# maximyudayev/Realtime-ST-GCN

Measured on AMD Instinct MI355X. Metric: skeleton-frames/sec/GPU (fwd+bwd), 10-layer ST-GCN N=64 T=300 V=25, higher is better.
Workload: dtype bf16; 1 GPU; config 2: as_is st-gcn (fcn_in + 9 StgcnLayer, BatchNorm, Kt=9), fwd + loss + bwd + Adam; global_batch=64, seq_len=300, joints=25, parallelism=single, bn_stats=per-replica, launch=eager

## Files before the change

realtime-st-gcn_amd/csrc/gconv.hip:

```cpp
#include "common.h"
#include "lds_ops.h"
#include "pack.h"
#include <stdlib.h>
#include "../../include/stgcn_amd.h"

#ifndef GCONV_NSTG_N
#define GCONV_NSTG_N 2
#endif
#ifndef GCONV_NSTG_M
#define GCONV_NSTG_M 2
#endif
#ifndef GCONV_NSTG_W
#define GCONV_NSTG_W 2
#endif
#ifndef GCONV_TM_W
#define GCONV_TM_W 2
#endif
#ifndef GCONV_TM_M
#define GCONV_TM_M 1
#endif

namespace {

template <typename T, int KC>
// ... 96 lines not shown
    const long joff = (long)src * a.in_ld + c * KC;
    const int ci = c * KC + ucol * VEC;
#pragma unroll
    for (int u = 0; u < A_UNITS; ++u) {
      ra[u] = make_uint4(0, 0, 0, 0);
      if (a_row[u] >= 0) {
        const T* p = in + a_row[u] + joff;
        if (fast_ld) {
          ra[u] = *reinterpret_cast<const uint4*>(p);
        } else if (ci < a.Cin) {
          float f[VEC];
#pragma unroll
          for (int e = 0; e < VEC; ++e) f[e] = ci + e < a.Cin ? Tr<T>::to_f(p[e]) : 0.f;
          ra[u] = pack16(f, (T*)nullptr);
        }
      }
    }
    char* B_ = smem + buf * STAGE + A_BYTES;
    const T* wsrc = wp + ((long)(jt * a.J + j) * a.Cout_pad + n0) * a.Cin_pad + c * KC;
#pragma unroll
    for (int kk = 0; kk < (B_PIECES + NW - 1) / NW; ++kk) {
      const int piece = wave + kk * NW;
      if (piece < B_PIECES) {
        const int byte = piece * 1024 + lane * 16;
        const int br = byte / L::RB, pu = (byte % L::RB) >> 4;
        glds16(wsrc + (long)br * a.Cin_pad + (pu ^ L::swz(br)) * VEC, B_ + piece * 1024);
      }
    }
  };
  auto store = [&](int buf) {
    char* A_ = smem + buf * STAGE;
#pragma unroll
    for (int u = 0; u < A_UNITS; ++u) *reinterpret_cast<uint4*>(A_ + a_lds[u]) = ra[u];
  };

  f32x16 acc[TM][TN];
#pragma unroll
  for (int i = 0; i < TM; ++i)
#pragma unroll
    for (int j = 0; j < TN; ++j)
#pragma unroll
      for (int r = 0; r < 16; ++r) acc[i][j][r] = 0.f;

  typedef typename Tr<T>::frag Frag;
  if constexpr (NSTG > 0) {
    static_assert(sizeof(T) == 2 && KC == 64, "DMA K loop: bf16, 64-channel chunks");
    constexpr int RBD = 128, A_B = BM * RBD, STG = A_B + BN * RBD;
    constexpr int AI = BM / 8 / NW, BI = BN / 8 / NW, OPS = AI + BI;
    static_assert(BM % (8 * NW) == 0 && BN % (8 * NW) == 0, "DMA rows");
    int* const snbr = reinterpret_cast<int*>(smem + NSTG * STG);
    if (tid < a.J) snbr[tid] = a.nbr[jt * a.J + tid];
    __syncthreads();
    const int rr = lane >> 3, slot = lane & 7;
    long a_src[AI];
    int b_src[BI];
#pragma unroll
    for (int q = 0; q < AI; ++q) {
      const int r = (wave * AI + q) * 8 + rr;
      const int rc = min(r, max(rows_valid, 1) - 1);
      a_src[q] = (long)(i0 + rc) * V * a.in_ld + (slot ^ ((r >> 1) & 7)) * 8;
    }
#pragma unroll
    for (int q = 0; q < BI; ++q) {
      const int r = (wave * BI + q) * 8 + rr;
      b_src[q] = (n0 + r) * a.Cin_pad + (slot ^ ((r >> 1) & 7)) * 8;
    }
    auto issue = [&](int k, int stage) {
      const int j = k / nch, c = k - j * nch;
      const long joff = (long)snbr[j] * a.in_ld + c * KC;
      const T* wsrc = wp + (long)(jt * a.J + j) * a.Cout_pad * a.Cin_pad + c * KC;
      char* base = smem + stage * STG;
#pragma unroll
      for (int q = 0; q < AI; ++q) glds16(in + a_src[q] + joff, lds_u32(base + (wave * AI + q) * 1024));
#pragma unroll
      for (int q = 0; q < BI; ++q) glds16(wsrc + b_src[q], lds_u32(base + A_B + (wave * BI + q) * 1024));
    };
#pragma unroll
    for (int sidx = 0; sidx < NSTG - 1; ++sidx)
      if (sidx < nk) issue(sidx, sidx);
    for (int k = 0; k < nk; ++k) {
      const int younger = min(NSTG - 2, nk - 1 - k);
      gwait_vm(younger * OPS);
      asm volatile("s_waitcnt lgkmcnt(0)\n\ts_barrier" ::: "memory");
      if (k + NSTG - 1 < nk) issue(k + NSTG - 1, (k + NSTG - 1) % NSTG);
      const char* A_ = smem + (k % NSTG) * STG;
      const char* B_ = A_ + A_B;
#pragma unroll
      for (int ks = 0; ks < KS; ++ks) {
        Frag fa[TM], fb[TN];
#pragma unroll
        for (int i = 0; i < TM; ++i) {
          const int r = (wm * TM + i) * 32 + lr;
          fa[i] = __builtin_bit_cast(bf16x8, *reinterpret_cast<const uint4*>(A_ + r * RBD + (((2 * ks + lh) ^ ((r >> 1) & 7)) << 4)));
        }
#pragma unroll
        for (int j = 0; j < TN; ++j) {
          const int r = (wn * TN + j) * 32 + lr;
          fb[j] = __builtin_bit_cast(bf16x8, *reinterpret_cast<const uint4*>(B_ + r * RBD + (((2 * ks + lh) ^ ((r >> 1) & 7)) << 4)));
        }
#pragma unroll
        for (int i = 0; i < TM; ++i)
#pragma unroll
          for (int j = 0; j < TN; ++j) Tr<T>::mma(acc[i][j], fa[i], fb[j]);
      }
    }
    __syncthreads();
  } else {
  int cur = 0;
  if (nk > 0) {
    load(0, 0);
    store(0);
  }
  __syncthreads();
  for (int k = 0; k < nk; ++k) {
    const bool more = k + 1 < nk;
    if (more) load(k + 1, cur ^ 1);
    const char* A_ = smem + cur * STAGE;
    const char* B_ = A_ + A_BYTES;
    Frag fa[2][TM], fb[2][TN];
    auto rd = [&](int ks, int b) {
#pragma unroll
      for (int i = 0; i < TM; ++i) {
        const char* p = A_ + a_off[i] + ks * 16 * (int)sizeof(T);
        fa[b][i] = frag2<T>(p, p + 16);
      }
#pragma unroll
      for (int j = 0; j < TN; ++j) {
        const char* p = B_ + ((wn * TN + j) * 32) * L::RB;
        fb[b][j] = frag2<T>(p + b_off[ks][0], p + b_off[ks][1]);
      }
    };
    rd(0, 0);
#pragma unroll
    for (int ks = 0; ks < KS; ++ks) {
      if (ks + 1 < KS) rd(ks + 1, (ks + 1) & 1);
#pragma unroll
      for (int i = 0; i < TM; ++i)
#pragma unroll
        for (int j = 0; j < TN; ++j) Tr<T>::mma(acc[i][j], fa[ks & 1][i], fb[ks & 1][j]);
      __builtin_amdgcn_sched_barrier(0);
    }
    if (more) store(cur ^ 1);
    __syncthreads();
    cur ^= 1;
  }
  }

  T* __restrict__ out = reinterpret_cast<T*>(a.out);
  const long ldv = (long)a.out_ld * V;
  constexpr int SROW = 32 * (int)sizeof(T) + 16;
  constexpr int UR = 32 * (int)sizeof(T) / 16;
  char* scratch = smem + wave * 32 * SROW;
  constexpr bool vec_out = ACCV;
  Welford ws[TN];
#pragma unroll
  for (int j = 0; j < TN; ++j) {
    const int c0 = n0 + (wn * TN + j) * 32;
    const int col = c0 + lr;
    const bool cok = col < a.Cout;
    const float b1 = (a.bias && cok) ? a.bias[jt * a.Cout + col] : 0.f;
    float s = 0.f, cnt = 0.f;
    if constexpr (!vec_out) {
#pragma unroll
      for (int i = 0; i < TM; ++i) {
        const int lb = (wm * TM + i) * 32 + 4 * lh;
        T* pb = out + ((long)(i0 + lb) * V + jt) * a.out_ld + col;
#pragma unroll
        for (int r = 0; r < 16; ++r) {
          const int ro = (r & 3) + 8 * (r >> 2);
          const bool ok = cok && lb + ro < rows_valid;
          float v = acc[i][j][r] + b1;
          if (ok) {
            T* p = pb + ro * ldv;
            if (a.accumulate) v += Tr<T>::to_f(*p);
            *p = Tr<T>::from_f(v);
            s += v;
            cnt += 1.f;
          }
          acc[i][j][r] = v;
        }
      }
    } else {
#pragma unroll
      for (int i = 0; i < TM; ++i) {
        const int rb = (wm * TM + i) * 32;
        const int lb = rb + 4 * lh;
#pragma unroll
        for (int r = 0; r < 16; ++r) {
          const int ro = (r & 3) + 8 * (r >> 2);
          const float v = acc[i][j][r] + b1;
          acc[i][j][r] = v;
          if (cok && lb + ro < rows_valid) {
            s += v;
            cnt += 1.f;
          }
          *reinterpret_cast<T*>(scratch + (4 * lh + ro) * SROW + lr * (int)sizeof(T)) = Tr<T>::from_f(v);
        }
#pragma unroll
        for (int q = 0; q < 32 * UR / 64; ++q) {
          const int idx = q * 64 + lane, row = idx / UR, u = idx % UR;
          if (rb + row < rows_valid && c0 + u * VEC < a.Cout) {
            T* p = out + ((long)(i0 + rb + row) * V + jt) * a.out_ld + c0 + u * VEC;
            float f[VEC], o[VEC];
            if (a.accumulate) {
              unpack16(*reinterpret_cast<const uint4*>(scratch + row * SROW + u * 16), f, (T*)nullptr);
              unpack16(*reinterpret_cast<const uint4*>(p), o, (T*)nullptr);
#pragma unroll
              for (int e = 0; e < VEC; ++e) f[e] += o[e];
              *reinterpret_cast<uint4*>(p) = pack16(f, (T*)nullptr);
            } else if (sizeof(T) == 2 && a.res) {
              const long grow = (long)(i0 + rb + row) * V + jt;
              const int cc = c0 + u * VEC;
              unpack16(*reinterpret_cast<const uint4*>(scratch + row * SROW + u * 16), f, (T*)nullptr);
              unpack16(*reinterpret_cast<const uint4*>(reinterpret_cast<const T*>(a.res) + grow * a.res_ld + cc), o,
                       (T*)nullptr);
              const unsigned mb = reinterpret_cast<const unsigned char*>(a.res_bits)[grow * (a.Cout / 8) + cc / 8];
#pragma unroll
              for (int e = 0; e < VEC; ++e) f[e] += ((mb >> e) & 1u) ? o[e] : 0.f;
              *reinterpret_cast<uint4*>(p) = pack16(f, (T*)nullptr);
            } else {
              *reinterpret_cast<uint4*>(p) = *reinterpret_cast<const uint4*>(scratch + row * SROW + u * 16);
            }
          }
        }
      }
    }
    Welford w;
    w.n = cnt;
    w.mean = cnt > 0.f ? s / cnt : 0.f;
    float m2 = 0.f;
    if (a.stats) {
#pragma unroll
      for (int i = 0; i < TM; ++i) {
        const int lb = (wm * TM + i) * 32 + 4 * lh;
#pragma unroll
        for (int r = 0; r < 16; ++r) {
          const float d = acc[i][j][r] - w.mean;
          if (cok && lb + (r & 3) + 8 * (r >> 2) < rows_valid) m2 += d * d;
        }
      }
    }
    w.m2 = m2;
    ws[j] = w;
  }
  if (a.stats) {
    __syncthreads();
    float4* red = reinterpret_cast<float4*>(smem);
#pragma unroll
    for (int j = 0; j < TN; ++j) {
      Welford o;
      o.n = __shfl_xor(ws[j].n, 32);
      o.mean = __shfl_xor(ws[j].mean, 32);
      o.m2 = __shfl_xor(ws[j].m2, 32);
      const Welford w = welford_merge(ws[j], o);
      if (lh == 0) red[wm * BN + (wn * TN + j) * 32 + lr] = make_float4(w.n, w.mean, w.m2, 0.f);
    }
    __syncthreads();
    for (int c = tid; c < BN; c += NT) {
      const float4 f = red[c];
      Welford w = {f.x, f.y, f.z};
      for (int k = 1; k < WM; ++k) {
        const float4 h = red[k * BN + c];
        w = welford_merge(w, Welford{h.x, h.y, h.z});
      }
      if (n0 + c < a.Cout_pad)
        reinterpret_cast<float4*>(a.stats)[((long)it * V + jt) * a.Cout_pad + n0 + c] =
            make_float4(w.n, w.mean, w.m2, 0.f);
    }
  }
}

template <typename T, int WM, int WN, int TM, int TN, int KC, int NSTG = 0>
int launch_gconv(const stgcn_gconv_desc& a, hipStream_t s) {
  constexpr int VEC = 16 / (int)sizeof(T);
  constexpr int BM = WM * TM * 32, BN = WN * TN * 32;
  typedef GL<T, KC> L;
  if (a.Cout_pad % BN || a.Cin_pad % KC) return STGCN_EBADSHAPE;
  if (NSTG && (a.in_ld % VEC || a.Cin != a.Cin_pad || a.J > 64)) return STGCN_EBADSHAPE;
  GGeom g;
  g.ntile = (a.NT + BM - 1) / BM;
  g.ncol = a.Cout_pad / BN;
  const long nblk = (long)g.ntile * a.V * g.ncol;
  if (nblk <= 0 || nblk > 0x7fffffffL) return STGCN_EBADSHAPE;
  g.nblk = (int)nblk;
  const int STAGE = ((BM * L::RS + BN * L::RB) + 1023) & ~1023;
  size_t lds = NSTG ? (size_t)NSTG * (BM + BN) * 128 + 256 : 2 * (size_t)STAGE;
  const size_t red = a.stats ? (size_t)WM * BN * 16 : 0;
  if (red > lds) lds = red;
  if (stgcn_lds_attr((const void*)gconv_kernel<T, WM, WN, TM, TN, KC, false, NSTG>, 160 * 1024, s) ||
      stgcn_lds_attr((const void*)gconv_kernel<T, WM, WN, TM, TN, KC, true, NSTG>, 160 * 1024, s))
    return STGCN_EHIP;
  const bool accv = (a.out_ld % VEC) == 0 && (a.Cout % VEC) == 0;
  if (a.res && (!accv || sizeof(T) != 2 || a.accumulate || !a.res_bits || a.Cout % 8 || a.res_ld % 8))
    return STGCN_EBADSHAPE;
  if (accv)
    hipLaunchKernelGGL((gconv_kernel<T, WM, WN, TM, TN, KC, true, NSTG>), dim3((unsigned)nblk), dim3(WM * WN * 64),
                       lds, s, a, g);
  else
    hipLaunchKernelGGL((gconv_kernel<T, WM, WN, TM, TN, KC, false, NSTG>), dim3((unsigned)nblk), dim3(WM * WN * 64),
                       lds, s, a, g);
  return hipGetLastError() == hipSuccess ? STGCN_OK : STGCN_EHIP;
}

template <typename T>
__global__ void gconv_weights_kernel(const float* __restrict__ A, const float* __restrict__ W, const int* nbr,
                                     const int* deg, int P, int V, int J, int Cout, int Cin, int trans, T* out,
                                     int R_pad, int C_pad, const float* __restrict__ bconv, float* __restrict__ bias2d) {
  __shared__ float colsum[GW_COLSUM_MAX];
  if (bias2d) gconv_colsum_block(A, nullptr, P, V, colsum);
  const long idx = (long)blockIdx.x * blockDim.x + threadIdx.x;
  if (idx < (long)V * R_pad * (C_pad / 8))
    gconv_weights_elem<T>(A, nullptr, W, nbr, deg, P, V, J, Cout, Cin, trans, out, R_pad, C_pad, bconv, bias2d, colsum,
                          idx);
}

constexpr int WKM = 128;
constexpr int WPR = 64;

struct WGG {
  int ntile, tpb, R, nco, nci;
  float* slab;
  float* rowpart;
  int zero_unused;
  float* part;
  unsigned* cnt;
};
constexpr int W3_SPLIT_DEG = 4;

__global__ __launch_bounds__(256, 2) void gconv_wgrad_kernel(const stgcn_gconv_wgrad_desc a, const WGG g) {
  constexpr int PANEL = WKM * WPR;
  constexpr int STAGE = 4 * PANEL;
  extern __shared__ __attribute__((aligned(16))) char smem[];
  const int tid = threadIdx.x, lane = tid & 63, wave = tid >> 6;
  const int V = a.V;
  const int ngrp = g.nco * g.nci;
  const int pair = blockIdx.x / (ngrp * g.R);
  const int rem = blockIdx.x % (ngrp * g.R);
  const int rr = rem / ngrp, grp = rem % ngrp;
  const int w = pair / a.J, j = pair % a.J;
  if (j >= a.deg[w]) return;
  const int src = a.nbr[pair];
  const int co0 = (grp % g.nco) * 64, ci0 = (grp / g.nco) * 64;
  const int t0 = rr * g.tpb, t1 = min(g.ntile, t0 + g.tpb);

  const bf16* __restrict__ dy = reinterpret_cast<const bf16*>(a.dy);
  const bf16* __restrict__ x = reinterpret_cast<const bf16*>(a.x);
  const int uc = tid & 7;
  const int co = co0 + uc * 8, ci = ci0 + uc * 8;
  uint4 ry[4], rx[4];
  auto load = [&](int t) {
#pragma unroll
    for (int u = 0; u < 4; ++u) {
      const int row = (tid >> 3) + u * 32;
      const int i = t * WKM + row;
      ry[u] = make_uint4(0, 0, 0, 0);
      rx[u] = make_uint4(0, 0, 0, 0);
      if (i < a.NT) {
        if (co < a.Cout) ry[u] = *reinterpret_cast<const uint4*>(dy + ((long)i * V + w) * a.dy_ld + co);
        if (ci < a.Cin) rx[u] = *reinterpret_cast<const uint4*>(x + ((long)i * V + src) * a.x_ld + ci);
      }
    }
  };
  auto store = [&](int buf) {
    char* base = smem + buf * STAGE;
#pragma unroll
    for (int u = 0; u < 4; ++u) {
      const int row = (tid >> 3) + u * 32;
      const int off = (uc >> 2) * PANEL + row * WPR + (uc & 3) * 16;
      *reinterpret_cast<uint4*>(base + off) = ry[u];
      *reinterpret_cast<uint4*>(base + 2 * PANEL + off) = rx[u];
    }
  };

  f32x16 acc[2][2];
#pragma unroll
  for (int a2 = 0; a2 < 2; ++a2)
#pragma unroll
    for (int b2 = 0; b2 < 2; ++b2)
#pragma unroll
      for (int r = 0; r < 16; ++r) acc[a2][b2][r] = 0.f;

  int cur = 0;
  if (t0 < t1) {
    load(t0);
    store(0);
  }
  __syncthreads();
  for (int t = t0; t < t1; ++t) {
    const bool more = t + 1 < t1;
    if (more) load(t + 1);
    const char* base = smem + cur * STAGE;
#pragma unroll
    for (int kk = 0; kk < WKM / 16 / 4; ++kk) {
      const int ks = wave + 4 * kk;
      bf16x8 fa[2], fb[2];
#pragma unroll
      for (int a2 = 0; a2 < 2; ++a2) fa[a2] = trfrag(base + a2 * PANEL, ks * 16, lane);
#pragma unroll
      for (int b2 = 0; b2 < 2; ++b2) fb[b2] = trfrag(base + (2 + b2) * PANEL, ks * 16, lane);
#pragma unroll
      for (int a2 = 0; a2 < 2; ++a2)
#pragma unroll
        for (int b2 = 0; b2 < 2; ++b2)
          acc[a2][b2] = __builtin_amdgcn_mfma_f32_32x32x16_bf16(fa[a2], fb[b2], acc[a2][b2], 0, 0, 0);
    }
    if (more) store(cur ^ 1);
    __syncthreads();
    cur ^= 1;
  }

  float* red = reinterpret_cast<float*>(smem);
  if (wave > 0) {
#pragma unroll
    for (int a2 = 0; a2 < 2; ++a2)
#pragma unroll
      for (int b2 = 0; b2 < 2; ++b2)
#pragma unroll
        for (int r = 0; r < 16; ++r) red[(((wave - 1) * 4 + a2 * 2 + b2) * 16 + r) * 64 + lane] = acc[a2][b2][r];
  }
  __syncthreads();
  if (wave == 0) {
    float* slab = g.slab + ((long)rr * V * a.J + pair) * a.Cout * a.Cin;
#pragma unroll
    for (int a2 = 0; a2 < 2; ++a2)
#pragma unroll
      for (int b2 = 0; b2 < 2; ++b2) {
        const int cc = ci0 + b2 * 32 + (lane & 31);
#pragma unroll
        for (int r = 0; r < 16; ++r) {
          float v = acc[a2][b2][r];
          for (int k = 0; k < 3; ++k) v += red[((k * 4 + a2 * 2 + b2) * 16 + r) * 64 + lane];
          const int oc = co0 + a2 * 32 + acc_row(r, lane);
          if (oc < a.Cout && cc < a.Cin) slab[(long)oc * a.Cin + cc] = v;
        }
      }
  }
}

constexpr int w2m(int cob) { return cob == 128 ? 64 : 32; }
constexpr int J2 = 5;
template <int COB>
__global__ __launch_bounds__(COB / 16 * 64, COB == 64 ? 3 : 1) void gconv_wgrad2_kernel(const stgcn_gconv_wgrad_desc a, const WGG g) {
  constexpr int NW = COB / 16, NT = NW * 64;
  constexpr int W2M = w2m(COB);
  constexpr int PANEL = W2M * WPR;
  constexpr int DYP = COB / 32;
  constexpr int STAGE = (DYP + 2 * J2) * PANEL;
  constexpr int DYU = COB * W2M / 8 / NT;
  constexpr int XU = 64 * W2M / 8 / NT;
  static_assert(DYU >= 1 && XU >= 1, "units");
  extern __shared__ __attribute__((aligned(16))) char smem[];
  const int tid = threadIdx.x, lane = tid & 63, wave = tid >> 6;
  const int cq = wave % DYP, ch = wave / DYP;
  const int V = a.V;
  const int ngrp = g.nco * g.nci;
  const int w = blockIdx.x / (ngrp * g.R);
  const int rem = blockIdx.x % (ngrp * g.R);
  const int rr = rem / ngrp, grp = rem % ngrp;
  const int deg = a.deg[w];
  const int co0 = (grp % g.nco) * COB, ci0 = (grp / g.nco) * 64;
  const int t0 = rr * g.tpb, t1 = min(g.ntile, t0 + g.tpb);
  int src[J2];
#pragma unroll
  for (int j = 0; j < J2; ++j) src[j] = j < deg ? a.nbr[w * a.J + j] : 0;

  const bf16* __restrict__ dy = reinterpret_cast<const bf16*>(a.dy);
  const bf16* __restrict__ x = reinterpret_cast<const bf16*>(a.x);
  uint4 ry[DYU], rx[J2][XU];
  auto load = [&](int t) {
#pragma unroll
    for (int u = 0; u < DYU; ++u) {
      const int e = tid + NT * u, row = e / (COB / 8), cu = e % (COB / 8);
      const int i = t * W2M + row;
      ry[u] = make_uint4(0, 0, 0, 0);
      if (i < a.NT && co0 + cu * 8 < a.Cout) ry[u] = *reinterpret_cast<const uint4*>(dy + ((long)i * V + w) * a.dy_ld + co0 + cu * 8);
    }
#pragma unroll
    for (int j = 0; j < J2; ++j)
#pragma unroll
      for (int u = 0; u < XU; ++u) {
        const int e = tid + NT * u, row = e >> 3, cu = e & 7;
        const int i = t * W2M + row;
        rx[j][u] = make_uint4(0, 0, 0, 0);
        if (j < deg && i < a.NT && ci0 + cu * 8 < a.Cin)
          rx[j][u] = *reinterpret_cast<const uint4*>(x + ((long)i * V + src[j]) * a.x_ld + ci0 + cu * 8);
      }
  };
  auto store = [&](int buf) {
    char* base = smem + buf * STAGE;
#pragma unroll
    for (int u = 0; u < DYU; ++u) {
      const int e = tid + NT * u, row = e / (COB / 8), cu = e % (COB / 8);
      *reinterpret_cast<uint4*>(base + (cu >> 2) * PANEL + row * WPR + (cu & 3) * 16) = ry[u];
    }
#pragma unroll
    for (int j = 0; j < J2; ++j)
#pragma unroll
      for (int u = 0; u < XU; ++u) {
        const int e = tid + NT * u, row = e >> 3, cu = e & 7;
        if (j < deg)
          *reinterpret_cast<uint4*>(base + (DYP + 2 * j + (cu >> 2)) * PANEL + row * WPR + (cu & 3) * 16) = rx[j][u];
      }
  };

  f32x16 acc[J2];
#pragma unroll
  for (int j = 0; j < J2; ++j)
#pragma unroll
    for (int r = 0; r < 16; ++r) acc[j][r] = 0.f;
  const bool rsum = g.rowpart != nullptr && grp / g.nco == 0;
  float sacc[DYU][8];
#pragma unroll
  for (int u = 0; u < DYU; ++u)
#pragma unroll
    for (int e = 0; e < 8; ++e) sacc[u][e] = 0.f;
  auto add_rows = [&]() {
    if (rsum) {
#pragma unroll
      for (int u = 0; u < DYU; ++u) {
        float f[8];
        unpack16(ry[u], f, (bf16*)nullptr);
#pragma unroll
        for (int e = 0; e < 8; ++e) sacc[u][e] += f[e];
      }
    }
  };

  int cur = 0;
  if (t0 < t1) {
    load(t0);
    add_rows();
    store(0);
  }
  __syncthreads();
  for (int t = t0; t < t1; ++t) {
    const bool more = t + 1 < t1;
    if (more) load(t + 1);
    const char* base = smem + cur * STAGE;
#pragma unroll
    for (int ks = 0; ks < W2M / 16; ++ks) {
      const bf16x8 fa = trfrag(base + cq * PANEL, ks * 16, lane);
#pragma unroll
      for (int j = 0; j < J2; ++j)
        if (j < deg) {
          const bf16x8 fb = trfrag(base + (DYP + 2 * j + ch) * PANEL, ks * 16, lane);
          acc[j] = __builtin_amdgcn_mfma_f32_32x32x16_bf16(fa, fb, acc[j], 0, 0, 0);
        }
    }
    if (more) {
      add_rows();
      store(cur ^ 1);
    }
    __syncthreads();
    cur ^= 1;
  }
  if (rsum) {
    float* red = reinterpret_cast<float*>(smem);
#pragma unroll
    for (int u = 0; u < DYU; ++u) {
      const int e = tid + NT * u, row = e / (COB / 8), cu = e % (COB / 8);
#pragma unroll
      for (int k = 0; k < 8; ++k) red[row * COB + cu * 8 + k] = sacc[u][k];
    }
    __syncthreads();
    if (tid < COB && co0 + tid < a.Cout) {
      float t = 0.f;
      for (int r = 0; r < W2M; ++r) t += red[r * COB + tid];
      g.rowpart[((long)rr * V + w) * a.Cout + co0 + tid] = t;
    }
  }

  const int cc = ci0 + ch * 32 + (lane & 31);
#pragma unroll
  for (int j = 0; j < J2; ++j) {
    if (j >= deg) continue;
    float* slab = g.slab + ((long)rr * V * a.J + w * a.J + j) * a.Cout * a.Cin;
#pragma unroll
    for (int r = 0; r < 16; ++r) {
      const int oc = co0 + cq * 32 + acc_row(r, lane);
      if (oc < a.Cout && cc < a.Cin) slab[(long)oc * a.Cin + cc] = acc[j][r];
    }
  }
}

constexpr int w3_stage(int deg) { return (2 + 2 * deg) * 32 * WPR; }
constexpr int w3d(int deg, int lds) { return lds / w3_stage(deg) > 8 ? 8 : lds / w3_stage(deg); }

template <int DEG, int LDSB>
DEV void wgrad3_body(const stgcn_gconv_wgrad_desc& a, const WGG& g, char* smem, int w, int rr, int grp, int t0,
                     int t1, int half) {
  constexpr int D = w3d(DEG, LDSB), PANEL = 32 * WPR, STAGE = w3_stage(DEG), NU = 1 + DEG;
  static_assert(D >= 3 && (D - 2) * NU <= 63, "ring");
  const int tid = threadIdx.x, lane = tid & 63, wave = __builtin_amdgcn_readfirstlane(tid >> 6);
  const int cq = wave & 1, ch = wave >> 1;
  const int V = a.V;
  const int co0 = (grp % g.nco) * 64, ci0 = (grp / g.nco) * 64;
  const bf16* __restrict__ dy = reinterpret_cast<const bf16*>(a.dy);
  const bf16* __restrict__ x = reinterpret_cast<const bf16*>(a.x);
  const int prow = 16 * (wave & 1) + (lane >> 2), pu = lane & 3, pp = wave >> 1;
  const bf16* ysrc = dy + (long)w * a.dy_ld + co0 + pp * 32 + pu * 8;
  const bf16* xsrc[DEG];
#pragma unroll
  for (int j = 0; j < DEG; ++j) xsrc[j] = x + (long)a.nbr[w * a.J + j] * a.x_ld + ci0 + pp * 32 + pu * 8;
  const long ystep = (long)V * a.dy_ld, xstep = (long)V * a.x_ld;
  const unsigned ring = lds_u32(smem);
  const unsigned woff = (unsigned)(pp * PANEL + (wave & 1) * 1024);
// ... 481 lines not shown
    float s = 0.f;
    if (pair % J < deg[pair / J])
      for (int r = 0; r < R; ++r) s += slab[(long)r * E + e];
    dweff[e] = s;
    return;
  }
  const long e = (long)(blockIdx.x - nb1) * blockDim.x + threadIdx.x;
  if (e >= ER) return;
  float s = 0.f;
  for (int r = 0; r < R; ++r) s += rpart[(long)r * ER + e];
  rowsum[e] = s;
}

__global__ void gslab_reduce_kernel(const float* __restrict__ slab, int R, long E, long EC, const int* deg, int J,
                                    float* __restrict__ out) {
  const long e = (long)blockIdx.x * blockDim.x + threadIdx.x;
  if (e >= E) return;
  const int pair = (int)(e / EC);
  float s = 0.f;
  if (pair % J < deg[pair / J])
    for (int r = 0; r < R; ++r) s += slab[(long)r * E + e];
  out[e] = s;
}

__global__ void gconv_dw_kernel(const float* __restrict__ dweff, const float* __restrict__ A, const int* nbr,
                                const int* deg, int P, int V, int J, int Cout, int Cin, float* dW) {
  const long idx = (long)blockIdx.x * blockDim.x + threadIdx.x;
  const long E = (long)Cout * Cin;
  if (idx >= (long)P * E) return;
  const int p = (int)(idx / E);
  const long e = idx % E;
  float s = 0.f;
  for (int w = 0; w < V; ++w)
    for (int j = 0; j < deg[w]; ++j) s += A[((long)p * V + nbr[w * J + j]) * V + w] * dweff[(long)(w * J + j) * E + e];
  dW[idx] += s;
}

__global__ void gconv_dA_kernel(const float* __restrict__ dweff, const float* __restrict__ W, const int* nbr,
                                const int* deg, int P, int V, int J, int Cout, int Cin, float* dA) {
  const int pair = blockIdx.x, p = blockIdx.y;
  const int w = pair / J, j = pair % J;
  if (j >= deg[w]) return;
  const long E = (long)Cout * Cin;
  const float* d = dweff + (long)pair * E;
  const float* wp = W + (long)p * E;
  float s = 0.f;
  for (long e = threadIdx.x; e < E; e += blockDim.x) s += wp[e] * d[e];
  s = wave_sum(s);
  __shared__ float part[4];
  if ((threadIdx.x & 63) == 0) part[threadIdx.x >> 6] = s;
  __syncthreads();
  if (threadIdx.x == 0) {
    const float t = part[0] + part[1] + part[2] + part[3];
    dA[((long)p * V + nbr[w * J + j]) * V + w] += t;
  }
}

constexpr int PMAX = 4;
constexpr int DW_PAIRS = 32 * 8;
DEV void gconv_dw_all_body(const float* __restrict__ dweff, const float* __restrict__ A, const int* nbr,
                           const int* deg, int P, int V, int J, long E, float* dW, long bb, bool acc_out) {
  __shared__ int spair[DW_PAIRS];
  __shared__ float scoef[DW_PAIRS][PMAX];
  __shared__ int snp;
  if (threadIdx.x == 0) {
    int n = 0;
    for (int w = 0; w < V; ++w)
      for (int j = 0; j < deg[w]; ++j) spair[n++] = w * J + j;
    snp = n;
  }
  __syncthreads();
  const int np = snp;
  for (int i = threadIdx.x; i < np * PMAX; i += 256) {
    const int k = i / PMAX, p = i % PMAX;
    const int pr = spair[k], w = pr / J;
    scoef[k][p] = p < P ? A[((long)p * V + nbr[pr]) * V + w] : 0.f;
  }
  __syncthreads();
  const int g = threadIdx.x >> 6;
  const long e = (bb * 64 + (threadIdx.x & 63)) * 4;
  float4 acc[PMAX];
#pragma unroll
  for (int p = 0; p < PMAX; ++p) acc[p] = make_float4(0.f, 0.f, 0.f, 0.f);
  if (e < E) {
#pragma unroll 4
    for (int k = g; k < np; k += 4) {
      const float4 d = *reinterpret_cast<const float4*>(dweff + (long)spair[k] * E + e);
#pragma unroll
      for (int p = 0; p < PMAX; ++p) {
        const float c = scoef[k][p];
        acc[p].x += c * d.x; acc[p].y += c * d.y; acc[p].z += c * d.z; acc[p].w += c * d.w;
      }
    }
  }
  __shared__ float4 part[4][PMAX][64];
#pragma unroll
  for (int p = 0; p < PMAX; ++p) part[g][p][threadIdx.x & 63] = acc[p];
  __syncthreads();
  if (threadIdx.x < 64 && e < E) {
    const int l = threadIdx.x;
#pragma unroll
    for (int p = 0; p < PMAX; ++p)
      if (p < P) {
        const float4 a0 = part[0][p][l], a1 = part[1][p][l], a2 = part[2][p][l], a3 = part[3][p][l];
        float4 t = make_float4(((a0.x + a1.x) + a2.x) + a3.x, ((a0.y + a1.y) + a2.y) + a3.y,
                               ((a0.z + a1.z) + a2.z) + a3.z, ((a0.w + a1.w) + a2.w) + a3.w);
        float4* o = reinterpret_cast<float4*>(dW + (long)p * E + e);
        if (acc_out) {
          const float4 q = *o;
          t.x += q.x; t.y += q.y; t.z += q.z; t.w += q.w;
        }
        *o = t;
      }
  }
}
__global__ __launch_bounds__(256) void gconv_dw_all_kernel(const float* __restrict__ dweff, const float* __restrict__ A,
                                                           const int* nbr, const int* deg, int P, int V, int J, long E,
                                                           float* dW) {
  gconv_dw_all_body(dweff, A, nbr, deg, P, V, J, E, dW, blockIdx.x, true);
}

constexpr int DA_CHUNK = 2048;
DEV void gconv_dA_part_body(const float* __restrict__ dweff, const float* __restrict__ W, const int* deg, int P, int J,
                           long E, float* part, int pair, int c, int nch) {
  if (pair % J >= deg[pair / J]) return;
  const float* d = dweff + (long)pair * E;
  float acc[PMAX] = {0.f, 0.f, 0.f, 0.f};
  const long e1 = min(E, (long)(c + 1) * DA_CHUNK);
  for (long e = (long)c * DA_CHUNK + threadIdx.x * 4; e < e1; e += 1024) {
    const float4 dv = *reinterpret_cast<const float4*>(d + e);
#pragma unroll
    for (int p = 0; p < PMAX; ++p)
      if (p < P) {
        const float4 w = *reinterpret_cast<const float4*>(W + (long)p * E + e);
        acc[p] += ((w.x * dv.x + w.y * dv.y) + w.z * dv.z) + w.w * dv.w;
      }
  }
  __shared__ float red[4][PMAX];
#pragma unroll
  for (int p = 0; p < PMAX; ++p) {
    const float t = wave_sum(acc[p]);
    if ((threadIdx.x & 63) == 0) red[threadIdx.x >> 6][p] = t;
  }
  __syncthreads();
  if (threadIdx.x < P)
    part[((long)pair * nch + c) * PMAX + threadIdx.x] =
        ((red[0][threadIdx.x] + red[1][threadIdx.x]) + red[2][threadIdx.x]) + red[3][threadIdx.x];
}
__global__ __launch_bounds__(256) void gconv_dA_part_kernel(const float* __restrict__ dweff, const float* __restrict__ W,
                                                            const int* deg, int P, int J, long E, float* part) {
  gconv_dA_part_body(dweff, W, deg, P, J, E, part, blockIdx.x, blockIdx.y, gridDim.y);
}

__global__ __launch_bounds__(256) void gconv_finish1_kernel(const float* __restrict__ dweff, const float* __restrict__ A,
                                                            const float* __restrict__ W, const int* nbr, const int* deg,
                                                            int P, int V, int J, long E, float* dW, int nb_dw, int nch,
                                                            float* part) {
  const int b = blockIdx.x;
  if (b < nb_dw) {
    gconv_dw_all_body(dweff, A, nbr, deg, P, V, J, E, dW, b, false);
  } else {
    const int b2 = b - nb_dw;
    gconv_dA_part_body(dweff, W, deg, P, J, E, part, b2 / nch, b2 % nch, nch);
  }
}

constexpr int FV_MAX = 32;
__global__ __launch_bounds__(256) void gconv_finish2_kernel(const float* __restrict__ part, const float* __restrict__ A,
                                                            const float* __restrict__ b, const float* __restrict__ S,
                                                            const int* nbr, const int* deg, int P, int V, int J, int C,
                                                            int nch, float* dA, float* db) {
  const int bx = blockIdx.x;
  if (bx < P * V) {
    const int p = bx / V, w = bx % V;
    float t = 0.f;
    for (int c = threadIdx.x; c < C; c += 256) t += b[p * C + c] * S[w * C + c];
    t = wave_sum(t);
    __shared__ float red[4];
    __shared__ float sup[FV_MAX];
    if ((threadIdx.x & 63) == 0) red[threadIdx.x >> 6] = t;
    if (threadIdx.x < V) sup[threadIdx.x] = 0.f;
    __syncthreads();
    const float tot = ((red[0] + red[1]) + red[2]) + red[3];
    if (threadIdx.x < deg[w]) {
      const int j = threadIdx.x, pair = w * J + j;
      float s = 0.f;
      for (int c = 0; c < nch; ++c) s += part[((long)pair * nch + c) * PMAX + p];
      sup[nbr[pair]] = s;
    }
    __syncthreads();
    for (int v = threadIdx.x; v < V; v += 256) dA[(p * V + v) * V + w] = sup[v] + tot;
    return;
  }
  __shared__ float cs[PMAX * FV_MAX];
  for (int i = threadIdx.x; i < P * V; i += 256) {
    const int p = i / V, w = i % V;
    float t = 0.f;
    for (int v = 0; v < V; ++v) t += A[(p * V + v) * V + w];
    cs[i] = t;
  }
  __syncthreads();
  const int i = (bx - P * V) * 256 + threadIdx.x;
  if (i >= P * C) return;
  const int p = i / C, c = i % C;
  float t = 0.f;
  for (int w = 0; w < V; ++w) t += cs[p * V + w] * S[w * C + c];
  db[i] = t;
}

__global__ void gconv_dA_reduce_kernel(const float* __restrict__ part, const int* nbr, const int* deg, int P, int V,
                                       int J, int nch, float* dA) {
  const int i = blockIdx.x * blockDim.x + threadIdx.x;
  if (i >= V * J * P) return;
  const int pair = i / P, p = i % P, w = pair / J, j = pair % J;
  if (j >= deg[w]) return;
  float s = 0.f;
  for (int c = 0; c < nch; ++c) s += part[((long)pair * nch + c) * PMAX + p];
  dA[((long)p * V + nbr[w * J + j]) * V + w] += s;
}

int w2_cob(const stgcn_gconv_wgrad_desc& a) {
  if (a.J > J2 || a.Cin % 64 || a.Cout % 64) return 0;
  return 64;
}

bool w3_ok(const stgcn_gconv_wgrad_desc& a) { return !(a.Cin == 64 && a.Cout == 128); }

#ifndef STGCN_W3_DEEP
#define STGCN_W3_DEEP 0
#endif
#ifndef STGCN_W3_WIDE_TARGET
#define STGCN_W3_WIDE_TARGET 256
#endif
WGG wplan2(const stgcn_gconv_wgrad_desc& a, int cob) {
  WGG g{};
  g.ntile = (a.NT + w2m(cob) - 1) / w2m(cob);
  g.nco = a.Cout / cob;
  g.nci = a.Cin / 64;
  const long groups = (long)a.V * g.nco * g.nci;
  const long target = cob == 64 ? 512 : 256;
#ifndef STGCN_W3_NARROW_TARGET
#define STGCN_W3_NARROW_TARGET 1024
#endif
  const long t3 = groups <= 32 ? STGCN_W3_NARROW_TARGET : groups < 200 ? 512 : STGCN_W3_WIDE_TARGET;
  long R = (cob == 64 && w3_ok(a)) ? (t3 + groups - 1) / groups : (target + groups - 1) / groups;
  if (R > g.ntile) R = g.ntile;
  if (R < 1) R = 1;
  g.tpb = (int)((g.ntile + R - 1) / R);
  g.R = (g.ntile + g.tpb - 1) / g.tpb;
  return g;
}

bool w3w_ok(const stgcn_gconv_wgrad_desc& a) {
  if (!STGCN_W3W || a.Cin % 128 || a.Cout % 128 || a.V > 64 || a.J > 2 * W3W_JE) return false;
  const long groups = (long)a.V * (a.Cout / 128) * (a.Cin / 128);
  return STGCN_W3W_TARGET / groups <= 2;
}
WGG wplan3w(const stgcn_gconv_wgrad_desc& a) {
  WGG g{};
  g.ntile = (a.NT + 31) / 32;
  g.nco = a.Cout / 128;
  g.nci = a.Cin / 128;
  const long groups = (long)a.V * g.nco * g.nci;
  long R = STGCN_W3W_TARGET / groups;
  if (R > g.ntile) R = g.ntile;
  if (R < 1) R = 1;
  g.tpb = (int)((g.ntile + R - 1) / R);
  g.R = (g.ntile + g.tpb - 1) / g.tpb;
  return g;
}
long w3w_part_floats(const stgcn_gconv_wgrad_desc& a, const WGG& g) {
  return g.R > 1 ? 2L * a.V * g.nco * g.nci * g.R * ((long)W3W_JE * W3W_PSZ_J + 128) : 0;
}
long w3w_cnt_bytes(const stgcn_gconv_wgrad_desc& a, const WGG& g) {
  return g.R > 1 ? ((2L * a.V * g.nco * g.nci * 4) + 15) / 16 * 16 : 0;
}

WGG wplan(const stgcn_gconv_wgrad_desc& a) {
  WGG g{};
  g.ntile = (a.NT + WKM - 1) / WKM;
  g.nco = (a.Cout + 63) / 64;
  g.nci = (a.Cin + 63) / 64;
  long used = 0;
  used = (long)a.V * a.J;
  const long groups = used * g.nco * g.nci;
  long R = (1024 + groups - 1) / groups;
  if (R > g.ntile) R = g.ntile;
  if (R < 1) R = 1;
  g.tpb = (int)((g.ntile + R - 1) / R);
  g.R = (g.ntile + g.tpb - 1) / g.tpb;
  return g;
}

}

long gconv_row_blocks(int NT, int V) { return (long)((NT + 127) / 128) * V; }

int gconv_launch(const stgcn_gconv_desc& a, int dtype, hipStream_t s) {
  const bool wide = a.Cout > 64;
  if (dtype == 1) {
    const bool dma = a.Cin % 64 == 0 && a.Cin == a.Cin_pad && a.in_ld % 8 == 0;
    if (dma) {
      if (!wide) return launch_gconv<bf16, 4, 1, 1, 2, 64, GCONV_NSTG_N>(a, s);
      return a.Cin >= 256 ? launch_gconv<bf16, 4, 2, GCONV_TM_W, 2, 64, GCONV_NSTG_W>(a, s)
                          : launch_gconv<bf16, 4, 2, GCONV_TM_M, 2, 64, GCONV_NSTG_M>(a, s);
    }
    const bool k64 = a.Cin >= 128 && a.Cin_pad % 64 == 0;
    if (wide) return k64 ? launch_gconv<bf16, 4, 2, 1, 2, 64>(a, s) : launch_gconv<bf16, 4, 2, 2, 2, 32>(a, s);
    return k64 ? launch_gconv<bf16, 4, 1, 1, 2, 64>(a, s) : launch_gconv<bf16, 4, 1, 1, 2, 32>(a, s);
  }
  return wide ? launch_gconv<float, 4, 2, 2, 2, 16>(a, s) : launch_gconv<float, 4, 1, 2, 2, 16>(a, s);
}

int gconv_weights_launch(const float* A, const float* W, const int* nbr, const int* deg, int P, int V, int J, int Cout,
                         int Cin, int trans, void* out, int R_pad, int C_pad, int dtype, hipStream_t s,
                         const float* bconv, float* bias2d) {
  if (C_pad % 8 || P > GW_PMAX || (bconv && P * V > GW_COLSUM_MAX)) return STGCN_EBADSHAPE;
  const long total = (long)V * R_pad * (C_pad / 8);
  const unsigned blocks = (unsigned)((total + 255) / 256);
  if (dtype == 1)
    hipLaunchKernelGGL(gconv_weights_kernel<bf16>, dim3(blocks), dim3(256), 0, s, A, W, nbr, deg, P, V, J, Cout, Cin,
                       trans, (bf16*)out, R_pad, C_pad, bconv, bias2d);
  else
    hipLaunchKernelGGL(gconv_weights_kernel<float>, dim3(blocks), dim3(256), 0, s, A, W, nbr, deg, P, V, J, Cout,
                       Cin, trans, (float*)out, R_pad, C_pad, bconv, bias2d);
  return hipGetLastError() == hipSuccess ? STGCN_OK : STGCN_EHIP;
}

long w3_split_part_floats(const stgcn_gconv_wgrad_desc& a, const WGG& g) {
  return (long)a.V * g.nco * g.nci * 2 * ((long)a.J * 4096 + 64);
}
long w3_split_cnt_bytes(const stgcn_gconv_wgrad_desc& a, const WGG& g) {
  return (((long)a.V * g.nco * g.nci * 4) + 15) / 16 * 16;
}

long gconv_wgrad_workspace(const stgcn_gconv_wgrad_desc& a, int dtype) {
  if (dtype != 1) return 0;
  const int cob = w2_cob(a);
  if (cob && w3w_ok(a)) {
    const WGG g = wplan3w(a);
    return w3w_part_floats(a, g) * (long)sizeof(float) + w3w_cnt_bytes(a, g);
  }
  const WGG g = cob ? wplan2(a, cob) : wplan(a);
  if (cob && w3_ok(a) && g.R == 1)
    return STGCN_W3_SPLIT ? w3_split_part_floats(a, g) * (long)sizeof(float) + w3_split_cnt_bytes(a, g) : 0;
  if (cob && a.rowsum)
    return ((long)g.R * a.V * a.J * a.Cout * a.Cin + (long)g.R * a.V * a.Cout) * (long)sizeof(float);
  return (long)g.R * a.V * a.J * a.Cout * a.Cin * (long)sizeof(float);
}

int gconv_wgrad_launch(const stgcn_gconv_wgrad_desc& a, int dtype, hipStream_t s) {
  const long E = (long)a.V * a.J * a.Cout * a.Cin;
  if (a.phase < 0 || a.phase > 2) return STGCN_EBADSHAPE;
  if (dtype != 1) {
    if (a.phase == 2) return STGCN_OK;
    hipLaunchKernelGGL(gconv_wgrad_f32_kernel, dim3((unsigned)((E + 255) / 256)), dim3(256), 0, s, a);
    return hipGetLastError() == hipSuccess ? STGCN_OK : STGCN_EHIP;
  }
  if (a.Cin % 8 || a.Cout % 8 || a.x_ld % 8 || a.dy_ld % 8) return STGCN_EBADSHAPE;
  const int cob = w2_cob(a);
  if (cob && w3w_ok(a)) {
    if (a.phase == 2) return STGCN_OK;
    WGG g = wplan3w(a);
    g.slab = a.dweff;
    g.rowpart = a.rowsum;
    g.zero_unused = 1;
    if (g.R > 1) {
      const long pf = w3w_part_floats(a, g), cb = w3w_cnt_bytes(a, g);
      if (!a.work || a.work_bytes < pf * (long)sizeof(float) + cb) return STGCN_EBADSHAPE;
      g.part = reinterpret_cast<float*>(a.work);
      g.cnt = reinterpret_cast<unsigned*>(g.part + pf);
      if (hipMemsetAsync(g.cnt, 0, (size_t)cb, s) != hipSuccess) return STGCN_EHIP;
    }
    if (stgcn_lds_attr((const void*)gconv_wgrad3w_kernel, W3W_LDS, s)) return STGCN_EHIP;
    const long blocks = 2L * a.V * g.nco * g.nci * g.R;
    hipLaunchKernelGGL(gconv_wgrad3w_kernel, dim3((unsigned)blocks), dim3(256), W3W_LDS, s, a, g);
    return hipGetLastError() == hipSuccess ? STGCN_OK : STGCN_EHIP;
  }
  if (cob) {
    WGG g = wplan2(a, cob);
    const bool ring = cob == 64 && w3_ok(a);
    const bool direct = ring && g.R == 1;
    const long need = (long)g.R * E + (a.rowsum ? (long)g.R * a.V * a.Cout : 0);
    if (direct) {
      g.slab = a.dweff;
      g.rowpart = a.rowsum;
      g.zero_unused = 1;
      if (STGCN_W3_SPLIT) {
        const long pf = w3_split_part_floats(a, g), cb = w3_split_cnt_bytes(a, g);
        if (!a.work || a.work_bytes < pf * (long)sizeof(float) + cb) return STGCN_EBADSHAPE;
        g.part = reinterpret_cast<float*>(a.work);
        g.cnt = reinterpret_cast<unsigned*>(g.part + pf);
        if (a.phase != 2 && hipMemsetAsync(g.cnt, 0, (size_t)cb, s) != hipSuccess) return STGCN_EHIP;
      }
    } else {
      if (!a.work || a.work_bytes < need * (long)sizeof(float)) return STGCN_EBADSHAPE;
      g.slab = reinterpret_cast<float*>(a.work);
      g.rowpart = a.rowsum ? g.slab + (long)g.R * E : nullptr;
    }
    const bool deep = (direct || STGCN_W3_DEEP > 1) && STGCN_W3_DEEP;
    const size_t lds = ring ? (size_t)(deep ? 160 : 80) * 1024 : 2 * (size_t)(cob / 32 + 2 * J2) * w2m(cob) * WPR;
    auto* k = ring ? (deep ? gconv_wgrad3_kernel<160 * 1024> : gconv_wgrad3_kernel<80 * 1024>) : gconv_wgrad2_kernel<64>;
    if (stgcn_lds_attr((const void*)k, 160 * 1024, s)) return STGCN_EHIP;
    const long blocks = (long)a.V * g.nco * g.nci * g.R * (g.part ? 2 : 1);
    if (a.phase != 2) hipLaunchKernelGGL(k, dim3((unsigned)blocks), dim3(ring ? 256 : cob / 16 * 64), lds, s, a, g);
    if (direct || a.phase == 1) return hipGetLastError() == hipSuccess ? STGCN_OK : STGCN_EHIP;
    if (a.rowsum) {
      const long ER = (long)a.V * a.Cout;
      const int nb1 = (int)((E + 255) / 256);
      hipLaunchKernelGGL(gslab_rowpart_kernel, dim3((unsigned)(nb1 + (ER + 255) / 256)), dim3(256), 0, s,
                         (const float*)g.slab, g.R, E, (long)a.Cout * a.Cin, a.deg, a.J, a.dweff, nb1,
                         (const float*)g.rowpart, ER, a.rowsum);
    } else {
      hipLaunchKernelGGL(gslab_reduce_kernel, dim3((unsigned)((E + 255) / 256)), dim3(256), 0, s, (const float*)g.slab,
                         g.R, E, (long)a.Cout * a.Cin, a.deg, a.J, a.dweff);
    }
    return hipGetLastError() == hipSuccess ? STGCN_OK : STGCN_EHIP;
  }
  if (a.rowsum) return STGCN_EBADSHAPE;
  WGG g = wplan(a);
  if (!a.work || a.work_bytes < (long)g.R * E * (long)sizeof(float)) return STGCN_EBADSHAPE;
  g.slab = reinterpret_cast<float*>(a.work);
  if (stgcn_lds_attr((const void*)gconv_wgrad_kernel, 160 * 1024, s)) return STGCN_EHIP;
  const long blocks = (long)a.V * a.J * g.nco * g.nci * g.R;
  const size_t lds = 2 * 4 * WKM * WPR;
  if (a.phase != 2) hipLaunchKernelGGL(gconv_wgrad_kernel, dim3((unsigned)blocks), dim3(256), lds, s, a, g);
  if (a.phase == 1) return hipGetLastError() == hipSuccess ? STGCN_OK : STGCN_EHIP;
  hipLaunchKernelGGL(gslab_reduce_kernel, dim3((unsigned)((E + 255) / 256)), dim3(256), 0, s, (const float*)g.slab,
                     g.R, E, (long)a.Cout * a.Cin, a.deg, a.J, a.dweff);
  return hipGetLastError() == hipSuccess ? STGCN_OK : STGCN_EHIP;
}

long gconv_wgrad_finish_workspace(int P, int V, int J, int Cout, int Cin) {
  const long E = (long)Cout * Cin;
  return P > PMAX ? 0 : (long)V * J * ((E + DA_CHUNK - 1) / DA_CHUNK) * PMAX * (long)sizeof(float);
}

bool gconv_finish_bias_ok(int P, int V, int J) { return P <= PMAX && V <= FV_MAX && V * J <= DW_PAIRS; }

int gconv_wgrad_finish_bias_launch(const float* dweff, const float* A, const float* W, const int* nbr, const int* deg,
                                   int P, int V, int J, int Cout, int Cin, const float* bconv, const float* S, float* dW,
                                   float* dA, float* db, void* work, hipStream_t s) {
  if (!gconv_finish_bias_ok(P, V, J) || !work || ((long)Cout * Cin) % 4) return STGCN_EBADSHAPE;
  const long E = (long)Cout * Cin;
  const int nch = (int)((E + DA_CHUNK - 1) / DA_CHUNK);
  const int nb_dw = (int)((E + 255) / 256);
  float* part = reinterpret_cast<float*>(work);
  hipLaunchKernelGGL(gconv_finish1_kernel, dim3((unsigned)(nb_dw + V * J * nch)), dim3(256), 0, s, dweff, A, W, nbr,
                     deg, P, V, J, E, dW, nb_dw, nch, part);
  hipLaunchKernelGGL(gconv_finish2_kernel, dim3((unsigned)(P * V + (P * Cout + 255) / 256)), dim3(256), 0, s,
                     (const float*)part, A, bconv, S, nbr, deg, P, V, J, Cout, nch, dA, db);
  return hipGetLastError() == hipSuccess ? STGCN_OK : STGCN_EHIP;
}

int gconv_wgrad_finish_launch(const float* dweff, const float* A, const float* W, const int* nbr, const int* deg,
                              int P, int V, int J, int Cout, int Cin, float* dW, float* dA, void* work, hipStream_t s) {
  const long E = (long)Cout * Cin;
  if (P > PMAX || (dA && !work) || V * J > DW_PAIRS || E % 4) {
    const long n = (long)P * E;
    if (dW)
      hipLaunchKernelGGL(gconv_dw_kernel, dim3((unsigned)((n + 255) / 256)), dim3(256), 0, s, dweff, A, nbr, deg, P,
                         V, J, Cout, Cin, dW);
    if (dA)
      hipLaunchKernelGGL(gconv_dA_kernel, dim3((unsigned)(V * J), (unsigned)P), dim3(256), 0, s, dweff, W, nbr, deg,
                         P, V, J, Cout, Cin, dA);
  } else {
    if (dW)
      hipLaunchKernelGGL(gconv_dw_all_kernel, dim3((unsigned)((E + 255) / 256)), dim3(256), 0, s, dweff, A, nbr, deg,
                         P, V, J, E, dW);
    if (dA) {
      const int nch = (int)((E + DA_CHUNK - 1) / DA_CHUNK);
      float* part = reinterpret_cast<float*>(work);
      hipLaunchKernelGGL(gconv_dA_part_kernel, dim3((unsigned)(V * J), (unsigned)nch), dim3(256), 0, s, dweff, W,
                         deg, P, J, E, part);
      hipLaunchKernelGGL(gconv_dA_reduce_kernel, dim3((unsigned)((V * J * P + 255) / 256)), dim3(256), 0, s, part,
                         nbr, deg, P, V, J, nch, dA);
    }
  }
  return hipGetLastError() == hipSuccess ? STGCN_OK : STGCN_EHIP;
}
```

Measured before the change: 2.537 million skeleton-frames/s.

## Add persistent graph-conv kernel with cross-tile prefetch for 256-channel layers

Adds a persistent bf16 graph-convolution kernel for layers with Cin>=256 and Cout_pad==256. It launches one block per CU, orders joints by degree to balance work, and prefetches the first K-chunk of the next tile while the current tile finishes, so the async-load pipeline stays full across tiles. It uses a larger 256x256 block tile with a fused bias, residual, accumulate and Welford-stats epilogue. The cost is one large block per CU with only double buffering, which lowers occupancy, and a new specialized code path to maintain.

After: 2.555 million skeleton-frames/s (median of 6 runs). Within noise of the previous version (+0.7%).

```diff
diff --git a/realtime-st-gcn_amd/csrc/gconv.hip b/realtime-st-gcn_amd/csrc/gconv.hip
--- a/realtime-st-gcn_amd/csrc/gconv.hip
+++ b/realtime-st-gcn_amd/csrc/gconv.hip
@@ -422,6 +422,263 @@
   return hipGetLastError() == hipSuccess ? STGCN_OK : STGCN_EHIP;
 }
 
+constexpr int GP_TAB = 128;
+constexpr int gp_epi_bytes(int bn) { return 8 * 32 * 80 > 4 * bn * 16 ? 8 * 32 * 80 : 4 * bn * 16; }
+
+__global__ __launch_bounds__(512, 1) void gconv_persist_kernel(const stgcn_gconv_desc a, const GGeom g) {
+  typedef bf16 T;
+  constexpr int WM = 4, WN = 2, TM = 2, TN = 4, NW = 8, NT = 512, KC = 64, KS = 4, VEC = 8;
+  constexpr int BM = WM * TM * 32, BN = WN * TN * 32;
+  constexpr int RBD = 128, A_B = BM * RBD, STG = A_B + BN * RBD, RING = 2 * STG;
+  constexpr int AI = BM / 8 / NW, BI = BN / 8 / NW;
+  extern __shared__ __attribute__((aligned(16))) char smem[];
+  char* const epi = smem + RING;
+  int* const ssj = reinterpret_cast<int*>(epi + gp_epi_bytes(BN));
+  int* const sdeg = ssj + 64;
+  int* const snbr = ssj + GP_TAB;
+  const int tid = threadIdx.x, lane = tid & 63, wave = __builtin_amdgcn_readfirstlane(tid >> 6);
+  const int wm = wave / WN, wn = wave % WN;
+  const int lr = lane & 31, lh = lane >> 5;
+  const int V = a.V, J = a.J;
+  const int nch = a.Cin_pad / KC;
+
+  for (int i = tid; i < V * J; i += NT) snbr[i] = a.nbr[i];
+  if (tid < V) {
+    const int d = a.deg[tid];
+    int rank = 0;
+    for (int v = 0; v < V; ++v) {
+      const int dv = a.deg[v];
+      rank += (dv > d || (dv == d && v < tid)) ? 1 : 0;
+    }
+    sdeg[tid] = d;
+    ssj[rank] = tid;
+  }
+  __syncthreads();
+
+  const int nitems = g.ntile * V;
+  int lb;
+  {
+    const int id = blockIdx.x, x = id & 7, q = g.nblk >> 3, r = g.nblk & 7;
+    lb = (x < r ? x * (q + 1) : r * (q + 1) + (x - r) * q) + (id >> 3);
+  }
+  auto item_at = [&](int r) -> int { return r * g.nblk + ((r & 1) ? g.nblk - 1 - lb : lb); };
+  if (lb >= nitems) return;
+
+  const T* __restrict__ in = reinterpret_cast<const T*>(a.in);
+  const T* __restrict__ wp = reinterpret_cast<const T*>(a.w);
+  T* __restrict__ out = reinterpret_cast<T*>(a.out);
+  const int rr = lane >> 3, slot = lane & 7;
+  long a_base = 0;
+  int a_src[AI];
+  auto aim = [&](int it) {
+    const int i0 = it * BM, rv = min(BM, a.NT - i0);
+    a_base = (long)i0 * V * a.in_ld;
+#pragma unroll
+    for (int q = 0; q < AI; ++q) {
+      const int r = (wave * AI + q) * 8 + rr;
+      const int rc = min(r, rv - 1);
+      a_src[q] = rc * V * a.in_ld + (slot ^ ((r >> 1) & 7)) * 8;
+    }
+  };
+  auto issue = [&](int jt, int k, int stage) {
+    const int j = k / nch, c = k - j * nch;
+    const int src = __builtin_amdgcn_readfirstlane(snbr[jt * J + j]);
+    const T* xsrc = in + a_base + (long)src * a.in_ld + c * KC;
+    const T* wsrc = wp + (long)(jt * J + j) * a.Cout_pad * a.Cin_pad + c * KC;
+    char* base = smem + stage * STG;
+#pragma unroll
+    for (int q = 0; q < AI; ++q) glds16(xsrc + a_src[q], lds_u32(base + (wave * AI + q) * 1024));
+#pragma unroll
+    for (int q = 0; q < BI; ++q) {
+      const int r = (wave * BI + q) * 8 + rr;
+      glds16(wsrc + r * a.Cin_pad + (slot ^ ((r >> 1) & 7)) * 8, lds_u32(base + A_B + (wave * BI + q) * 1024));
+    }
+  };
+
+  constexpr int SROW = 32 * (int)sizeof(T) + 16;
+  constexpr int UR = 32 * (int)sizeof(T) / 16;
+  char* const scratch = epi + wave * 32 * SROW;
+
+  int stage = 0;
+  bool primed = false;
+  for (int round = 0;; ++round) {
+    const int pos = item_at(round);
+    if (pos >= nitems) break;
+    const int jt = __builtin_amdgcn_readfirstlane(ssj[pos / g.ntile]), it = pos % g.ntile;
+    const int nk = __builtin_amdgcn_readfirstlane(sdeg[jt]) * nch;
+    const int i0 = it * BM;
+    const int rows_valid = min(BM, a.NT - i0);
+    if (!primed && nk > 0) {
+      aim(it);
+      issue(jt, 0, stage);
+    }
+    primed = false;
+
+    f32x16 acc[TM][TN];
+#pragma unroll
+    for (int i = 0; i < TM; ++i)
+#pragma unroll
+      for (int j = 0; j < TN; ++j)
+#pragma unroll
+        for (int r = 0; r < 16; ++r) acc[i][j][r] = 0.f;
+
+    for (int k = 0; k < nk; ++k) {
+      asm volatile("s_waitcnt vmcnt(0)" ::: "memory");
+      lds_barrier();
+      if (k + 1 < nk) {
+        issue(jt, k + 1, stage ^ 1);
+      } else if (item_at(round + 1) < nitems) {
+        const int pos2 = item_at(round + 1);
+        const int jt2 = __builtin_amdgcn_readfirstlane(ssj[pos2 / g.ntile]), it2 = pos2 % g.ntile;
+        if (__builtin_amdgcn_readfirstlane(sdeg[jt2]) > 0) {
+          aim(it2);
+          issue(jt2, 0, stage ^ 1);
+          primed = true;
+        }
+      }
+      const char* A_ = smem + stage * STG;
+      const char* B_ = A_ + A_B;
+#pragma unroll
+      for (int ks = 0; ks < KS; ++ks) {
+        bf16x8 fa[TM], fb[TN];
+#pragma unroll
+        for (int i = 0; i < TM; ++i) {
+          const int r = (wm * TM + i) * 32 + lr;
+          fa[i] = __builtin_bit_cast(bf16x8, *reinterpret_cast<const uint4*>(A_ + r * RBD + (((2 * ks + lh) ^ ((r >> 1) & 7)) << 4)));
+        }
+#pragma unroll
+        for (int j = 0; j < TN; ++j) {
+          const int r = (wn * TN + j) * 32 + lr;
+          fb[j] = __builtin_bit_cast(bf16x8, *reinterpret_cast<const uint4*>(B_ + r * RBD + (((2 * ks + lh) ^ ((r >> 1) & 7)) << 4)));
+        }
+#pragma unroll
+        for (int i = 0; i < TM; ++i)
+#pragma unroll
+          for (int j = 0; j < TN; ++j) Tr<T>::mma(acc[i][j], fa[i], fb[j]);
+      }
+      stage ^= 1;
+    }
+
+    int el = lane;
+    asm volatile("" : "+v"(el));
+    const int lr = el & 31, lh = el >> 5;
+    Welford ws[TN];
+#pragma unroll
+    for (int j = 0; j < TN; ++j) {
+      const int c0 = (wn * TN + j) * 32;
+      const int col = c0 + lr;
+      const bool cok = col < a.Cout;
+      const float b1 = (a.bias && cok) ? a.bias[jt * a.Cout + col] : 0.f;
+      float s = 0.f, cnt = 0.f;
+#pragma unroll
+      for (int i = 0; i < TM; ++i) {
+        const int rb = (wm * TM + i) * 32;
+        const int lb4 = rb + 4 * lh;
+#pragma unroll
+        for (int r = 0; r < 16; ++r) {
+          const int ro = (r & 3) + 8 * (r >> 2);
+          const float v = acc[i][j][r] + b1;
+          acc[i][j][r] = v;
+          if (cok && lb4 + ro < rows_valid) {
+            s += v;
+            cnt += 1.f;
+          }
+          *reinterpret_cast<T*>(scratch + (4 * lh + ro) * SROW + lr * (int)sizeof(T)) = Tr<T>::from_f(v);
+        }
+#pragma unroll
+        for (int q = 0; q < 32 * UR / 64; ++q) {
+          const int idx = q * 64 + el, row = idx / UR, u = idx % UR;
+          if (rb + row < rows_valid && c0 + u * VEC < a.Cout) {
+            T* p = out + ((long)(i0 + rb + row) * V + jt) * a.out_ld + c0 + u * VEC;
+            float f[VEC], o[VEC];
+            if (a.accumulate) {
+              unpack16(*reinterpret_cast<const uint4*>(scratch + row * SROW + u * 16), f, (T*)nullptr);
+              unpack16(*reinterpret_cast<const uint4*>(p), o, (T*)nullptr);
+#pragma unroll
+              for (int e = 0; e < VEC; ++e) f[e] += o[e];
+              *reinterpret_cast<uint4*>(p) = pack16(f, (T*)nullptr);
+            } else if (a.res) {
+              const long grow = (long)(i0 + rb + row) * V + jt;
+              const int cc = c0 + u * VEC;
+              unpack16(*reinterpret_cast<const uint4*>(scratch + row * SROW + u * 16), f, (T*)nullptr);
+              unpack16(*reinterpret_cast<const uint4*>(reinterpret_cast<const T*>(a.res) + grow * a.res_ld + cc), o,
+                       (T*)nullptr);
+              const unsigned mb = reinterpret_cast<const unsigned char*>(a.res_bits)[grow * (a.Cout / 8) + cc / 8];
+#pragma unroll
+              for (int e = 0; e < VEC; ++e) f[e] += ((mb >> e) & 1u) ? o[e] : 0.f;
+              *reinterpret_cast<uint4*>(p) = pack16(f, (T*)nullptr);
+            } else {
+              *reinterpret_cast<uint4*>(p) = *reinterpret_cast<const uint4*>(scratch + row * SROW + u * 16);
+            }
+          }
+        }
+      }
+      Welford w;
+      w.n = cnt;
+      w.mean = cnt > 0.f ? s / cnt : 0.f;
+      float m2 = 0.f;
+      if (a.stats) {
+#pragma unroll
+        for (int i = 0; i < TM; ++i) {
+          const int lb4 = (wm * TM + i) * 32 + 4 * lh;
+#pragma unroll
+          for (int r = 0; r < 16; ++r) {
+            const float d = acc[i][j][r] - w.mean;
+            if (cok && lb4 + (r & 3) + 8 * (r >> 2) < rows_valid) m2 += d * d;
+          }
+        }
+      }
+      w.m2 = m2;
+      ws[j] = w;
+    }
+    if (a.stats) {
+      lds_barrier();
+      float4* red = reinterpret_cast<float4*>(epi);
+#pragma unroll
+      for (int j = 0; j < TN; ++j) {
+        Welford o;
+        o.n = __shfl_xor(ws[j].n, 32);
+        o.mean = __shfl_xor(ws[j].mean, 32);
+        o.m2 = __shfl_xor(ws[j].m2, 32);
+        const Welford w = welford_merge(ws[j], o);
+        if (lh == 0) red[wm * BN + (wn * TN + j) * 32 + lr] = make_float4(w.n, w.mean, w.m2, 0.f);
+      }
+      lds_barrier();
+      for (int c = wave * 64 + el; c < BN; c += NT) {
+        const float4 f = red[c];
+        Welford w = {f.x, f.y, f.z};
+        for (int k = 1; k < WM; ++k) {
+          const float4 h = red[k * BN + c];
+          w = welford_merge(w, Welford{h.x, h.y, h.z});
+        }
+        if (c < a.Cout_pad)
+          reinterpret_cast<float4*>(a.stats)[((long)it * V + jt) * a.Cout_pad + c] = make_float4(w.n, w.mean, w.m2, 0.f);
+      }
+      lds_barrier();
+    }
+  }
+}
+
+int launch_gconv_persist(const stgcn_gconv_desc& a, hipStream_t s, bool* taken) {
+  constexpr int BN = 256;
+  *taken = false;
+  const bool accv = (a.out_ld % 8) == 0 && (a.Cout % 8) == 0;
+  const size_t lds = 2 * (size_t)(256 + BN) * 128 + gp_epi_bytes(BN) + ((size_t)GP_TAB + (size_t)a.V * a.J) * 4;
+  const long nitems = (long)((a.NT + 255) / 256) * a.V;
+  if (a.Cout_pad != BN || a.Cin_pad % 64 || a.Cin != a.Cin_pad || a.in_ld % 8 || a.in_ld > 65536 || !accv ||
+      a.V > 64 || a.J > 64 || lds > 160 * 1024 || nitems <= 0 || nitems > 0x3fffffffL)
+    return STGCN_OK;
+  *taken = true;
+  if (a.res && (a.accumulate || !a.res_bits || a.Cout % 8 || a.res_ld % 8)) return STGCN_EBADSHAPE;
+  GGeom g;
+  g.ntile = (a.NT + 255) / 256;
+  g.ncol = 1;
+  g.nblk = stgcn_cu_count(s);
+  if (stgcn_lds_attr((const void*)gconv_persist_kernel, 160 * 1024, s)) return STGCN_EHIP;
+  hipLaunchKernelGGL((gconv_persist_kernel), dim3((unsigned)g.nblk), dim3(512), lds, s, a, g);
+  return hipGetLastError() == hipSuccess ? STGCN_OK : STGCN_EHIP;
+}
+
 template <typename T>
 __global__ void gconv_weights_kernel(const float* __restrict__ A, const float* __restrict__ W, const int* nbr,
                                      const int* deg, int P, int V, int J, int Cout, int Cin, int trans, T* out,
@@ -1509,6 +1766,11 @@
     const bool dma = a.Cin % 64 == 0 && a.Cin == a.Cin_pad && a.in_ld % 8 == 0;
     if (dma) {
       if (!wide) return launch_gconv<bf16, 4, 1, 1, 2, 64, GCONV_NSTG_N>(a, s);
+      if (a.Cin >= 256 && a.Cout_pad == 256) {
+        bool taken = false;
+        const int rc = launch_gconv_persist(a, s, &taken);
+        if (taken) return rc;
+      }
       return a.Cin >= 256 ? launch_gconv<bf16, 4, 2, GCONV_TM_W, 2, 64, GCONV_NSTG_W>(a, s)
                           : launch_gconv<bf16, 4, 2, GCONV_TM_M, 2, 64, GCONV_NSTG_M>(a, s);
     }
```
